# DidItWork/Sigma-Zero

Measured on AMD Instinct MI355X. Metric: MCTS simulations/sec (self-play), higher is better.
Workload: dtype bf16

## Files before the change

### sigma-zero_amd/csrc/sz_nn.hip

```cpp
#include "sz_nn_common.h"

#ifndef NN_EXPLICIT_WAIT
#define NN_EXPLICIT_WAIT 2
#endif
#ifndef NN_TAPGAP
#define NN_TAPGAP 1
#endif


template <int CIN, int NTAPS, int WGB, bool PROBE16 = false>
__device__ __forceinline__ void conv_kloop(const unsigned char* lds, const uint4* __restrict__ w, f32x16 (&acc)[NN_NI][2 * WGB], bool skip) {
    constexpr int PITCH = CIN * 2 + 16;
    constexpr int KSTEPS = CIN / 16;
    constexpr int ZERO_ROW = WGB * 64;
    constexpr int NI = NN_NI, NJ = 2 * WGB;
    constexpr int RING = 4, PF = RING - 1;
    constexpr int TOTAL_KS = NTAPS * KSTEPS;
    constexpr int W_KSTEP_STRIDE = 8 * 64;
    const int lane = threadIdx.x & 63, wave = threadIdx.x >> 6;
    const int p32 = lane & 31, h = lane >> 5;
    const uint4* wbase = w + (size_t)(wave * NI) * 64 + lane;
#pragma unroll
    for (int i = 0; i < NI; i++)
#pragma unroll
        for (int j = 0; j < NJ; j++)
#pragma unroll
            for (int r = 0; r < 16; r++) acc[i][j][r] = 0.f;
    uint4 aring[RING][NI];
#pragma unroll
    for (int s = 0; s < PF; s++)
#pragma unroll
        for (int i = 0; i < NI; i++) aring[s][i] = wbase[(size_t)s * W_KSTEP_STRIDE + i * 64];
    auto tap_addr = [&](int tap, int j) -> int {
        const int dy = (NTAPS == 9) ? tap / 3 - 1 : 0, dx = (NTAPS == 9) ? tap % 3 - 1 : 0;
        int pos = (j & 1) * 32 + p32;
        int y = (pos >> 3) + dy, x = (pos & 7) + dx;
        bool ok = (unsigned)y < 8u && (unsigned)x < 8u;
        int row = ok ? ((j >> 1) * 64 + y * 8 + x) : ZERO_ROW;
        return row * PITCH + h * 16;
    };
    int bcur[NJ], bnxt[NJ];
    bf16x8 bfrag[2][NJ];
#pragma unroll
    for (int j = 0; j < NJ; j++) { bcur[j] = tap_addr(0, j); bnxt[j] = bcur[j]; bfrag[0][j] = *(const bf16x8*)(lds + bcur[j]); }
    for (int tap = 0; tap < (skip ? 0 : NTAPS); tap++) {
        if (tap + 1 < NTAPS) {
#pragma unroll
            for (int j = 0; j < NJ; j++) bnxt[j] = tap_addr(tap + 1, j);
        }
#pragma unroll
        for (int kc = 0; kc < KSTEPS; kc++) {
            const int ks = tap * KSTEPS + kc;
            if (ks + PF < TOTAL_KS) {
#pragma unroll
                for (int i = 0; i < NI; i++) aring[(kc + PF) & (RING - 1)][i] = wbase[(size_t)(ks + PF) * W_KSTEP_STRIDE + i * 64];
            }
            if (kc + 1 < KSTEPS) {
#pragma unroll
                for (int j = 0; j < NJ; j++) bfrag[(kc + 1) & 1][j] = *(const bf16x8*)(lds + bcur[j] + (kc + 1) * 32);
            } else if (tap + 1 < NTAPS) {
#pragma unroll
                for (int j = 0; j < NJ; j++) bfrag[(kc + 1) & 1][j] = *(const bf16x8*)(lds + bnxt[j]);
            }
            asm volatile("" ::: "memory");
            __builtin_amdgcn_sched_barrier(0);
#pragma unroll
            for (int i = 0; i < NI; i++) {
                bf16x8 a = __builtin_bit_cast(bf16x8, aring[kc & (RING - 1)][i]);
#pragma unroll
                for (int j = 0; j < NJ; j++) {
                    if constexpr (PROBE16) {
#pragma unroll
                        for (int q = 0; q < 2; q++) {
                            f32x4 c4 = {acc[i][j][8 * q], acc[i][j][8 * q + 1], acc[i][j][8 * q + 2], acc[i][j][8 * q + 3]};
                            c4 = __builtin_amdgcn_mfma_f32_16x16x32_bf16(a, bfrag[kc & 1][j], c4, 0, 0, 0);
                            acc[i][j][8 * q] = c4[0]; acc[i][j][8 * q + 1] = c4[1]; acc[i][j][8 * q + 2] = c4[2]; acc[i][j][8 * q + 3] = c4[3];
                        }
                    } else {
                        acc[i][j] = __builtin_amdgcn_mfma_f32_32x32x16_bf16(a, bfrag[kc & 1][j], acc[i][j], 0, 0, 0);
                    }
                }
            }
            __builtin_amdgcn_sched_barrier(0);
        }
#pragma unroll
        for (int j = 0; j < NJ; j++) bcur[j] = bnxt[j];
    }
}

template <int WGB>
__device__ __forceinline__ void acc_to_lds(unsigned char* lds, const f32x16 (&acc)[NN_NI][2 * WGB], const float* __restrict__ bias, bool relu) {
    constexpr int OPITCH = NN_COUT * 2 + 16;
    const int lane = threadIdx.x & 63, wave = threadIdx.x >> 6;
    const int p32 = lane & 31, h = lane >> 5;
#pragma unroll
    for (int j = 0; j < 2 * WGB; j++) {
        const int row = (j >> 1) * 64 + (j & 1) * 32 + p32;
#pragma unroll
        for (int i = 0; i < NN_NI; i++) {
#pragma unroll
            for (int g = 0; g < 4; g++) {
                const int co = (wave * NN_NI + i) * 32 + 8 * g + 4 * h;
                f32x4 b4 = *(const f32x4*)(bias + co);
                float v0 = acc[i][j][4 * g + 0] + b4[0], v1 = acc[i][j][4 * g + 1] + b4[1];
                float v2 = acc[i][j][4 * g + 2] + b4[2], v3 = acc[i][j][4 * g + 3] + b4[3];
                if (relu) { v0 = fmaxf(v0, 0.f); v1 = fmaxf(v1, 0.f); v2 = fmaxf(v2, 0.f); v3 = fmaxf(v3, 0.f); }
                uint2 o; o.x = pack_bf16x2(v0, v1); o.y = pack_bf16x2(v2, v3);
                *(uint2*)(lds + row * OPITCH + co * 2) = o;
            }
        }
    }
}

template <int WGB, int PAD = 16, bool NT = false, bool NTS = NT>
__device__ __forceinline__ void lds_to_out(const unsigned char* lds, const uint16_t* __restrict__ res, uint16_t* __restrict__ out, int board0, int n_boards, bool relu) {
    constexpr int OPITCH = NN_COUT * 2 + PAD;
    constexpr int OUT_CHUNKS = WGB * 64 * 32;
    const int tid = threadIdx.x;
    const int valid = min(WGB, n_boards - board0) * 64 * 32;
    const uint4* res4 = res ? (const uint4*)(res + (size_t)board0 * 64 * NN_COUT) : nullptr;
    uint4* out4 = (uint4*)(out + (size_t)board0 * 64 * NN_COUT);
#pragma unroll 4
    for (int c = tid; c < OUT_CHUNKS; c += 256) {
        if (c >= valid) break;
        uint4 v = *(const uint4*)(lds + (c >> 5) * OPITCH + (c & 31) * 16);
        if (!res4 && !relu) {
            if (NTS) st_stream(out4 + c, v); else out4[c] = v;
            continue;
        }
        float f[8] = {bf16_lo(v.x), bf16_hi(v.x), bf16_lo(v.y), bf16_hi(v.y), bf16_lo(v.z), bf16_hi(v.z), bf16_lo(v.w), bf16_hi(v.w)};
        if (res4) {
            uint4 r = NT ? ld_stream(res4 + c) : res4[c];
            f[0] += bf16_lo(r.x); f[1] += bf16_hi(r.x); f[2] += bf16_lo(r.y); f[3] += bf16_hi(r.y);
            f[4] += bf16_lo(r.z); f[5] += bf16_hi(r.z); f[6] += bf16_lo(r.w); f[7] += bf16_hi(r.w);
        }
        if (relu) {
#pragma unroll
            for (int k = 0; k < 8; k++) f[k] = fmaxf(f[k], 0.f);
        }
        uint4 o;
        o.x = pack_bf16x2(f[0], f[1]); o.y = pack_bf16x2(f[2], f[3]); o.z = pack_bf16x2(f[4], f[5]); o.w = pack_bf16x2(f[6], f[7]);
        if (NTS) st_stream(out4 + c, o); else out4[c] = o;
    }
}


template <int RING>
__device__ __forceinline__ void conv_prefetch16(const uint4* __restrict__ w, uint4 (&aring)[RING][4]) {
    const int lane = threadIdx.x & 63, wave = threadIdx.x >> 6;
    const uint32_t wlane = (uint32_t)((wave * 4) * 64 + lane) * 16u;
    const WSrc wr = wfrag_rsrc(w);
#pragma unroll
    for (int s = 0; s < RING - 1; s++)
#pragma unroll
        for (int i = 0; i < 4; i++) aring[s][i] = ld_wfrag(wr, (size_t)s * (16 * 64), wlane + i * 1024);
    asm volatile("" ::: "memory");
    __builtin_amdgcn_sched_barrier(0);
}


template <int CIN, int NTAPS, int WGB, int RING = 2, bool PREFETCHED = false, int ABL = 0 ,
          bool ACCUM = false ,
          class E = ElemBF16 ,
          class EPI = std::nullptr_t >
__device__ __forceinline__ void conv_kloop16(const unsigned char* lds, const uint4* __restrict__ w, f32x4 (&acc)[4][4 * WGB], bool skip, bool wprobe = false,
                                             uint4 (*ring_in)[4] = nullptr, const int img_off = 0 ,
                                             const float* __restrict__ bias = nullptr ,
                                             const int* addr_tab = nullptr ,
                                             EPI epi0 = EPI()) {
    constexpr int PITCH = CIN * 2 + NN_PAD16;
    constexpr int KSTEPS = CIN / 32;
    constexpr int NI = 4, NJ = 4 * WGB, NH = NJ / 2;
    constexpr int TOTAL_KS = NTAPS * KSTEPS;
    const int W_KSTEP_STRIDE = wprobe ? 0 : 16 * 64;
    const int lane = threadIdx.x & 63, wave = threadIdx.x >> 6;
    const int p16 = lane & 15, kg = lane >> 4;
    const uint32_t wlane = (uint32_t)((wave * NI) * 64 + lane) * 16u;
    const WSrc wr = wfrag_rsrc(w);
    f32x4 binit[NI];
#pragma unroll
    for (int i = 0; i < NI; i++) binit[i] = bias ? *(const f32x4*)(bias + (wave * NI + i) * 16 + 4 * kg) : f32x4{0.f, 0.f, 0.f, 0.f};
    constexpr bool PEEL = RING == 4;
    constexpr bool SKIPROWS = PEEL && NTAPS == 9 && WGB == 2 && !(ABL & 4) && NN_ROWSKIP;
    if ((skip || !PEEL) && !ACCUM) {
#pragma unroll
        for (int i = 0; i < NI; i++)
#pragma unroll
            for (int j = 0; j < NJ; j++) acc[i][j] = binit[i];
    } else if (SKIPROWS && !ACCUM) {
#pragma unroll
        for (int i = 0; i < NI; i++) acc[i][0] = binit[i];
    }
    constexpr int PF = RING - 1;
    static_assert(KSTEPS % RING == 0, "ring slots must be compile-time indices");
    uint4 aring[RING][NI];
#pragma unroll
    for (int s = 0; s < PF; s++)
#pragma unroll
        for (int i = 0; i < NI; i++) {
            if constexpr (PREFETCHED) aring[s][i] = ring_in[s][i];
            else aring[s][i] = ld_wfrag(wr, (size_t)s * W_KSTEP_STRIDE, wlane + i * 1024);
        }
    auto tap_addr = [&](int tap, int j) -> int {
        return addr_tab ? addr_tab[(tap * NJ + j) * 64 + lane] : conv_tap_addr16<PITCH, NTAPS, WGB>(tap, j, p16, kg);
    };
    constexpr int TABPITCH = NN_COUT * 2 + NN_PAD16;
    constexpr bool CONVERT = PITCH != TABPITCH;
    auto tab_convert = [&](int rel) -> int {
        if constexpr (!CONVERT) return rel;
        else {
            const int row = (int)__umulhi((unsigned)rel, 7895161u);
            return rel >= WGB * 64 * TABPITCH ? rel - WGB * 64 * (TABPITCH - PITCH) : rel - row * (TABPITCH - PITCH);
        }
    };
    const int lds_base = (int)(uint32_t)(uintptr_t)lds;
    auto abs_addr = [&](int rel) -> int {
        int a = lds_base + img_off + rel;
        asm volatile("" : "+v"(a));
        return a;
    };
    auto LD = [](int addr) -> bf16x8 { return *(const __attribute__((address_space(3))) bf16x8*)(uint32_t)addr; };
    int bcur[NJ], bnxt[NJ];
    bf16x8 bfrag[2][NH];
#pragma unroll
    for (int j = 0; j < NJ; j++) { bnxt[j] = addr_tab ? tab_convert(tap_addr(0, j)) : tap_addr(0, j); bcur[j] = abs_addr(bnxt[j]); }
#pragma unroll
    for (int j = 0; j < NH; j++)
        if (!(SKIPROWS && j == 0)) bfrag[0][j] = LD(bcur[j]);
    auto tap_body = [&](const int tap, auto first_tag, auto skip_tag) {
        constexpr bool FIRST = decltype(first_tag)::value;
        constexpr int SK = decltype(skip_tag)::value;
        constexpr bool TAPGAP = NN_TAPGAP && PEEL && NN_ILV && NH + NJ <= NI * (NH - 1);
        const bool in_gaps = TAPGAP && addr_tab != nullptr;
        if (tap + 1 < NTAPS && !in_gaps) {
#pragma unroll
            for (int j = 0; j < NJ; j++) bnxt[j] = addr_tab ? tab_convert(tap_addr(tap + 1, j)) : tap_addr(tap + 1, j);
        }
#pragma unroll
        for (int kc = 0; kc < KSTEPS; kc++) {
            const int ks = tap * KSTEPS + kc;
#pragma unroll
            for (int hs = 0; hs < 2; hs++) {
                if (!NN_ILV) {
                    if (hs == 0 && ks + PF < TOTAL_KS) {
#pragma unroll
                        for (int i = 0; i < NI; i++) aring[(kc + PF) & (RING - 1)][i] = ld_wfrag(wr, (size_t)(ks + PF) * W_KSTEP_STRIDE, wlane + i * 1024);
                    }
                    if (hs == 0) {
#pragma unroll
                        for (int j = 0; j < NH; j++) if (!(SK == 2 && j == NH - 1)) bfrag[1][j] = LD(bcur[NH + j] + kc * 64);
                    } else if (kc + 1 < KSTEPS) {
#pragma unroll
                        for (int j = 0; j < NH; j++) if (!(SK == 1 && j == 0)) bfrag[0][j] = LD(bcur[j] + (kc + 1) * 64);
                    } else if (tap + 1 < NTAPS) {
#pragma unroll
                        for (int j = 0; j < NH; j++) if (!(SK == 1 && j == 0 && tap + 1 < 3)) bfrag[0][j] = LD(abs_addr(bnxt[j]));
                    }
                    asm volatile("" ::: "memory");
                    __builtin_amdgcn_sched_barrier(0);
                }
#pragma unroll
                for (int i = 0; i < NI; i++) {
                    bf16x8 a = __builtin_bit_cast(bf16x8, aring[kc & (RING - 1)][i]);
#pragma unroll
                    for (int j = 0; j < NH; j++) {
                        const bool idle_hs = (SK == 1 && hs == 0) || (SK == 2 && hs == 1);
                        const bool idle = idle_hs && j == (SK == 1 ? 0 : NH - 1);
                        if (!idle) acc[i][hs * NH + j] = E::mfma(a, bfrag[hs][j], (FIRST && kc == 0) ? binit[i] : acc[i][hs * NH + j]);
                        if (NN_ILV && !idle) {
                            const int NR = idle_hs ? NH - 1 : NH, m = i * NR + (idle_hs && SK == 1 ? j - 1 : j);
                            if (m < NH) {
                                if ((ABL & 2) || (SK == 2 && hs == 0 && m == NH - 1)) {}
                                else if (hs == 0) bfrag[1][m] = LD(bcur[NH + m] + kc * 64);
                                else if (kc + 1 < KSTEPS) { if (!(SK == 1 && m == 0)) bfrag[0][m] = LD(bcur[m] + (kc + 1) * 64); }
                                else if (tap + 1 < NTAPS) { if (!(SK == 1 && m == 0 && tap + 1 < 3)) bfrag[0][m] = LD(abs_addr(bnxt[m])); }
                            } else if (m < NH + NI && hs == 0) {
                                if (ABL & 1) {}
                                else if (ks + PF < TOTAL_KS)
                                    aring[(kc + PF) & (RING - 1)][m - NH] = ld_wfrag(wr, (size_t)(ks + PF) * W_KSTEP_STRIDE, wlane + (m - NH) * 1024);
                            } else if (TAPGAP && hs == 1 && m >= NH && m < NH + NJ) {
                                if (in_gaps) {
                                    if (kc == 0) bnxt[m - NH] = tap_addr(tap + 1 < NTAPS ? tap + 1 : tap, m - NH);
                                    else if (CONVERT && kc == 1) bnxt[m - NH] = tab_convert(bnxt[m - NH]);
                                    else if (kc == KSTEPS - 1) bcur[m - NH] = abs_addr(bnxt[m - NH]);
                                }
                            }
#if NN_EXPLICIT_WAIT
                            if (PEEL && m == NI * NR - 1) {
                                if (NN_EXPLICIT_WAIT >= 2 && hs == 1) __builtin_amdgcn_s_waitcnt(0x0078);
                                else __builtin_amdgcn_s_waitcnt(0xC07F);
                            }
#endif
                            asm volatile("" ::: "memory");
                            __builtin_amdgcn_sched_barrier(0);
                        }
                    }
                }
                __builtin_amdgcn_sched_barrier(0);
            }
        }
        if (!in_gaps) {
#pragma unroll
            for (int j = 0; j < NJ; j++) bcur[j] = abs_addr(bnxt[j]);
        }
    };
    constexpr bool SPLIT = !std::is_same<EPI, std::nullptr_t>::value && NTAPS == 9 && NN_ILV && PEEL && KSTEPS % RING == 0;
    auto last_tap_split = [&]() {
        if constexpr (SPLIT) {
            constexpr int tap = NTAPS - 1;
#pragma unroll
            for (int kc = 0; kc < KSTEPS; kc++) {
                const int ks = tap * KSTEPS + kc;
#pragma unroll
                for (int i = 0; i < NI; i++) {
                    bf16x8 a = __builtin_bit_cast(bf16x8, aring[kc & (RING - 1)][i]);
#pragma unroll
                    for (int j = 0; j < NH; j++) {
                        acc[i][j] = E::mfma(a, bfrag[kc & 1][j], acc[i][j]);
                        const int m = i * NH + j;
                        if (m < NH) {
                            if (ABL & 2) {}
                            else if (kc + 1 < KSTEPS) bfrag[(kc + 1) & 1][m] = LD(bcur[m] + (kc + 1) * 64);
                            else if (!(SKIPROWS && m == NH - 1)) bfrag[(kc + 1) & 1][m] = LD(bcur[NH + m]);
                        } else if (m < NH + NI) {
                            const int vks = ks + PF, wks = vks < TOTAL_KS ? vks : vks - KSTEPS;
                            if (!(ABL & 1)) aring[(kc + PF) & (RING - 1)][m - NH] = ld_wfrag(wr, (size_t)wks * W_KSTEP_STRIDE, wlane + (m - NH) * 1024);
                        } else if (kc == KSTEPS - 1 && (m == 2 * NH || m == 3 * NH)) {
                            epi0(m == 2 * NH ? 0 : 1, -1);
                        }
#if NN_EXPLICIT_WAIT >= 2
                        if (m == NI * NH - 1) __builtin_amdgcn_s_waitcnt(0x0078);
#endif
                        asm volatile("" ::: "memory");
                        __builtin_amdgcn_sched_barrier(0);
                    }
                }
            }
#pragma unroll
            for (int kc = 0; kc < KSTEPS; kc++) {
#pragma unroll
                for (int i = 0; i < NI; i++) {
                    bf16x8 a = __builtin_bit_cast(bf16x8, aring[kc & (RING - 1)][i]);
#pragma unroll
                    for (int j = 0; j < NH; j++) {
                        if (!(SKIPROWS && j == NH - 1))
                            acc[i][NH + j] = E::mfma(a, bfrag[kc & 1][j], acc[i][NH + j]);
                        const int m = i * NH + j;
                        if (m < NH) {
                            if (!(ABL & 2) && kc + 1 < KSTEPS && !(SKIPROWS && m == NH - 1)) bfrag[(kc + 1) & 1][m] = LD(bcur[NH + m] + (kc + 1) * 64);
                        } else if (m < NH + NI) {
                            if (!(ABL & 1) && kc + PF < KSTEPS)
                                aring[(kc + PF) & (RING - 1)][m - NH] = ld_wfrag(wr, (size_t)(tap * KSTEPS + kc + PF) * W_KSTEP_STRIDE, wlane + (m - NH) * 1024);
                        } else {
                            const int p = 2 * kc + (m >= 3 * NH ? 1 : 0);
                            if (p < NI * NH) epi0(p, (m - 2 * NH) & 3);
                        }
                        asm volatile("" ::: "memory");
                        __builtin_amdgcn_sched_barrier(0);
                    }
                }
            }
        }
    };
    if (!skip) {
        using SK0 = std::integral_constant<int, 0>;
        if constexpr (SKIPROWS) {
            using SK1 = std::integral_constant<int, 1>; using SK2 = std::integral_constant<int, 2>;
            tap_body(0, std::integral_constant<bool, !ACCUM>{}, SK1{});
            for (int tap = 1; tap < 3; tap++) tap_body(tap, std::false_type{}, SK1{});
            for (int tap = 3; tap < 6; tap++) tap_body(tap, std::false_type{}, SK0{});
            for (int tap = 6; tap < (SPLIT ? NTAPS - 1 : NTAPS); tap++) tap_body(tap, std::false_type{}, SK2{});
            last_tap_split();
        } else if constexpr (PEEL) {
            tap_body(0, std::integral_constant<bool, !ACCUM>{}, SK0{});
            for (int tap = 1; tap < (SPLIT ? NTAPS - 1 : NTAPS); tap++) tap_body(tap, std::false_type{}, SK0{});
            last_tap_split();
        } else {
            for (int tap = 0; tap < NTAPS; tap++) tap_body(tap, std::false_type{}, SK0{});
        }
    }
}

#ifndef NN_ONE_RING
#define NN_ONE_RING 4
#endif
#ifndef NN_ONE_WHOT
#define NN_ONE_WHOT 0
#endif
template <int ABL = 0, class E = ElemBF16>
__device__ __forceinline__ void conv_kloop16_one(const unsigned char* lds, const uint4* __restrict__ w, f32x4 (&acc)[4][4], uint4 (*ring_in)[4] , const int img_off,
                                                 const float* __restrict__ bias, const int* addr_tab) {
    constexpr int KSTEPS = NN_COUT / 32, NI = 4, NJ = 4, NTAPS = 9, RING = NN_ONE_RING, PF = RING - 1, TOTAL_KS = NTAPS * KSTEPS;
    constexpr int W_KSTEP_STRIDE = NN_ONE_WHOT ? 0 : 16 * 64;
    static_assert(KSTEPS % RING == 0, "ring slots must be compile-time indices");
    const int lane = threadIdx.x & 63, wave = threadIdx.x >> 6, kg = lane >> 4;
    const uint32_t wlane = (uint32_t)((wave * NI) * 64 + lane) * 16u;
    const WSrc wr = wfrag_rsrc(w);
    f32x4 binit[NI];
#pragma unroll
    for (int i = 0; i < NI; i++) binit[i] = *(const f32x4*)(bias + (wave * NI + i) * 16 + 4 * kg);
    uint4 aring[RING][NI];
#pragma unroll
    for (int s_ = 0; s_ < PF; s_++)
#pragma unroll
        for (int i = 0; i < NI; i++) aring[s_][i] = ring_in[s_][i];
    const int lds_base = (int)(uint32_t)(uintptr_t)lds;
    auto abs_addr = [&](int rel) -> int {
        int a = lds_base + img_off + rel;
        asm volatile("" : "+v"(a));
        return a;
    };
    auto LD = [](int addr) -> bf16x8 { return *(const __attribute__((address_space(3))) bf16x8*)(uint32_t)addr; };
    int bcur[NJ], bnxt[NJ];
    bf16x8 bfrag[2][NJ];
#pragma unroll
    for (int j = 0; j < NJ; j++) { bnxt[j] = addr_tab[j * 64 + lane]; bcur[j] = abs_addr(bnxt[j]); }
#pragma unroll
    for (int j = 0; j < NJ; j++) bfrag[0][j] = LD(bcur[j]);
    auto tap_body = [&](const int tap, auto first_tag) {
        constexpr bool FIRST = decltype(first_tag)::value;
#pragma unroll
        for (int kc = 0; kc < KSTEPS; kc++) {
            const int ks = tap * KSTEPS + kc;
#pragma unroll
            for (int i = 0; i < NI; i++) {
                const bf16x8 a = __builtin_bit_cast(bf16x8, aring[kc & (RING - 1)][i]);
#pragma unroll
                for (int j = 0; j < NJ; j++) {
                    acc[i][j] = E::mfma(a, bfrag[kc & 1][j], (FIRST && kc == 0) ? binit[i] : acc[i][j]);
                    const int m = i * NJ + j;
                    if (m < NJ) {
                        if (ABL & 2) {}
                        else if (kc + 1 < KSTEPS) bfrag[(kc + 1) & 1][m] = LD(bcur[m] + (kc + 1) * 64);
                        else if (tap + 1 < NTAPS) bfrag[(kc + 1) & 1][m] = LD(abs_addr(bnxt[m]));
                    } else if (m < NJ + NI) {
                        if (!(ABL & 1) && ks + PF < TOTAL_KS)
                            aring[(kc + PF) & (RING - 1)][m - NJ] = ld_wfrag(wr, (size_t)(ks + PF) * W_KSTEP_STRIDE, wlane + (m - NJ) * 1024);
                    } else if (m < 2 * NJ + NI) {
                        if (kc == 0) bnxt[m - NJ - NI] = addr_tab[((tap + 1 < NTAPS ? tap + 1 : tap) * NJ + (m - NJ - NI)) * 64 + lane];
                        else if (kc == KSTEPS - 1) bcur[m - NJ - NI] = abs_addr(bnxt[m - NJ - NI]);
                    } else if (m == NI * NJ - 1) {
                        if (RING == 4) __builtin_amdgcn_s_waitcnt(0x0078);
                        else __builtin_amdgcn_s_waitcnt(0x4078);
                    }
                    asm volatile("" ::: "memory");
                    __builtin_amdgcn_sched_barrier(0);
                }
            }
        }
    };
    tap_body(0, std::true_type{});
    for (int tap = 1; tap < NTAPS; tap++) tap_body(tap, std::false_type{});
}

#ifndef NN_EPI_NOCONFLICT
#define NN_EPI_NOCONFLICT 0
#endif
__device__ __forceinline__ int epi_slot16(int row, int co) {
#if NN_EPI_NOCONFLICT
    return ((row >> 3) & 7) * 8192 + (co >> 2) * 128 + (((row >> 6) << 3) | (row & 7)) * 8;
#else
    return row * (NN_COUT * 2 + NN_PAD16) + co * 2;
#endif
}

template <int WGB, class E = ElemBF16> struct EpiTile16 {
    unsigned char* img; const f32x4 (&acc)[4][4 * WGB]; f32x4 tv; uint2 o;
    __device__ __forceinline__ EpiTile16(unsigned char* img_, const f32x4 (&acc_)[4][4 * WGB]) : img(img_), acc(acc_) {}
    __device__ __forceinline__ void operator()(int p, int st) {
        const int i = p / (2 * WGB), j = p % (2 * WGB);
        if (st == 0) tv = acc[i][j];
        else if (st == 1) o.x = relu_bf16x2(E::pack2(tv[0], tv[1]));
        else if (st == 2) o.y = relu_bf16x2(E::pack2(tv[2], tv[3]));
        else if (st == 3) {
            const int lane = threadIdx.x & 63, wave = threadIdx.x >> 6;
            const int row = tile_row<WGB>(j, lane & 15), co = (wave * 4 + i) * 16 + 4 * (lane >> 4);
            *(uint2*)(img + epi_slot16(row, co)) = o;
        }
    }
};
template <int WGB, class E = ElemBF16> struct EpiResidual16 {
    unsigned char* img; const f32x4 (&acc)[4][4 * WGB]; f32x4 tv; uint2 o; uint2 rr[3];
    __device__ __forceinline__ EpiResidual16(unsigned char* img_, const f32x4 (&acc_)[4][4 * WGB]) : img(img_), acc(acc_) {}
    __device__ __forceinline__ uint2* slot(int p) const {
        const int i = p / (2 * WGB), j = p % (2 * WGB);
        const int lane = threadIdx.x & 63, wave = threadIdx.x >> 6;
        const int row = tile_row<WGB>(j, lane & 15), co = (wave * 4 + i) * 16 + 4 * (lane >> 4);
        return (uint2*)(img + epi_slot16(row, co));
    }
    __device__ __forceinline__ void operator()(int p, int st) {
        const int i = p / (2 * WGB), j = p % (2 * WGB);
        if (st == -1) rr[p % 3] = *slot(p);
        else if (st == 0) { tv = acc[i][j]; if (p + 2 < 8 * WGB) rr[(p + 2) % 3] = *slot(p + 2); }
        else if (st == 1) o.x = relu_bf16x2(E::pack2(tv[0] + E::lo(rr[p % 3].x), tv[1] + E::hi(rr[p % 3].x)));
        else if (st == 2) o.y = relu_bf16x2(E::pack2(tv[2] + E::lo(rr[p % 3].y), tv[3] + E::hi(rr[p % 3].y)));
        else if (st == 3) *slot(p) = o;
    }
};

template <int WGB, class E = ElemBF16>
__device__ __forceinline__ void acc_tile_to_lds16(unsigned char* lds, const f32x4 (&acc)[4][4 * WGB], int i, int j, bool relu) {
    constexpr int OPITCH = NN_COUT * 2 + NN_PAD16;
    const int lane = threadIdx.x & 63, wave = threadIdx.x >> 6;
    const int row = tile_row<WGB>(j, lane & 15), co = (wave * 4 + i) * 16 + 4 * (lane >> 4);
    const f32x4 v = acc[i][j];
    uint2 o;
    o.x = E::pack2(v[0], v[1]);
    o.y = E::pack2(v[2], v[3]);
    if (relu) { o.x = relu_bf16x2(o.x); o.y = relu_bf16x2(o.y); }
    *(uint2*)(lds + epi_slot16(row, co)) = o;
}
template <int WGB, class E = ElemBF16>
__device__ __forceinline__ void acc_tile_residual16(unsigned char* xlds, const f32x4 (&acc)[4][4 * WGB], int i, int j) {
    constexpr int OPITCH = NN_COUT * 2 + NN_PAD16;
    const int lane = threadIdx.x & 63, wave = threadIdx.x >> 6;
    const int row = tile_row<WGB>(j, lane & 15), co = (wave * 4 + i) * 16 + 4 * (lane >> 4);
    const f32x4 v = acc[i][j];
    uint2* px = (uint2*)(xlds + epi_slot16(row, co));
    const uint2 r = *px;
    uint2 o;
    o.x = relu_bf16x2(E::pack2(v[0] + E::lo(r.x), v[1] + E::hi(r.x)));
    o.y = relu_bf16x2(E::pack2(v[2] + E::lo(r.y), v[3] + E::hi(r.y)));
    *px = o;
}

template <int WGB, class E = ElemBF16>
__device__ __forceinline__ void acc_to_lds16(unsigned char* lds, const f32x4 (&acc)[4][4 * WGB], const float* __restrict__ bias, bool relu) {
    constexpr int OPITCH = NN_COUT * 2 + NN_PAD16;
    const int lane = threadIdx.x & 63, wave = threadIdx.x >> 6;
    const int p16 = lane & 15, kg = lane >> 4;
#pragma unroll
    for (int j = 0; j < 4 * WGB; j++) {
        const int row = tile_row<WGB>(j, p16);
#pragma unroll
        for (int i = 0; i < 4; i++) {
            const int co = (wave * 4 + i) * 16 + 4 * kg;
            f32x4 v = acc[i][j];
            if (bias) v += *(const f32x4*)(bias + co);
            uint2 o;
            o.x = E::pack2(v[0], v[1]);
            o.y = E::pack2(v[2], v[3]);
            if (relu) { o.x = relu_bf16x2(o.x); o.y = relu_bf16x2(o.y); }
            *(uint2*)(lds + row * OPITCH + co * 2) = o;
        }
    }
}

__device__ __forceinline__ void phase_stagger(int flags, int n_cu) {
    const int stagger = (flags >> 8) & 0xFF;
    if (!stagger) return;
    bool second = false;
    if (flags & 32) second = ((int)blockIdx.x >= n_cu && (int)blockIdx.x < 2 * n_cu);
    if (flags & 64) second = ((int)blockIdx.x < 2 * n_cu) && ((__builtin_amdgcn_s_getreg(0x1804) & 1) != 0);
    if (__builtin_amdgcn_readfirstlane((int)second))
        for (int i = 0; i < stagger; i++) __builtin_amdgcn_s_sleep(127);
}

template <int CIN, int NTAPS, int WGB >
__global__ __launch_bounds__(256, (WGB == 2 ? 2 : 1)) void k_conv_bf16(const uint16_t* __restrict__ in, const uint4* __restrict__ w, const float* __restrict__ bias,
                                                      const uint16_t* __restrict__ res, uint16_t* __restrict__ out, int n_boards, int flags, int n_cu) {
    extern __shared__ __attribute__((aligned(16))) unsigned char lds[];
    const int board0 = blockIdx.x * WGB;
    stage_tile<CIN, WGB>(lds, in, board0, n_boards, (flags & 2) != 0);
    __syncthreads();
    if (WGB == 2) phase_stagger(flags, n_cu);
    f32x16 acc[NN_NI][2 * WGB];
    if (CIN == 256 && NTAPS == 9 && WGB == 2 && (flags & 0x20000)) conv_kloop<CIN, NTAPS, WGB, true>(lds, w, acc, (flags & 8) != 0);
    else conv_kloop<CIN, NTAPS, WGB>(lds, w, acc, (flags & 8) != 0);
    __syncthreads();
    if (!((flags & 4) && acc[0][0][0] != 12345.f)) acc_to_lds<WGB>(lds, acc, bias, false);
    __syncthreads();
    if (!(flags & 4)) lds_to_out<WGB>(lds, res, out, board0, n_boards, (flags & 1) != 0);
}

template <int WGB>
__global__ __launch_bounds__(256, (WGB == 2 ? 2 : 1)) void k_block_bf16(const uint16_t* __restrict__ in, const uint4* __restrict__ w1, const float* __restrict__ b1,
                                                       const uint4* __restrict__ w2, const float* __restrict__ b2, uint16_t* __restrict__ out,
                                                       int n_boards, int flags, int n_cu) {
    extern __shared__ __attribute__((aligned(16))) unsigned char lds[];
// ... 277 lines not shown
    float inv = 1.0f;
    if (do_softmax) {
        for (int off = 32; off >= 1; off >>= 1) mx = fmaxf(mx, __shfl_xor(mx, off));
        if (lane == 0) red[wave * 2] = mx;
        __syncthreads();
        mx = fmaxf(red[wave * 2], red[(wave ^ 1) * 2]);
        float sum = 0.f;
#pragma unroll
        for (int i = 0; i < 5; i++)
#pragma unroll
            for (int r = 0; r < 4; r++) {
                const int co = i * 16 + 4 * kg + r;
#pragma unroll
                for (int j = 0; j < 2; j++) {
                    const float e = co < 73 ? __expf(pa[i][j][r] - mx) : 0.f;
                    pa[i][j][r] = e;
                    sum += e;
                }
            }
        for (int off = 32; off >= 1; off >>= 1) sum += __shfl_xor(sum, off);
        if (lane == 0) red[wave * 2 + 1] = sum;
        __syncthreads();
        inv = 1.0f / (red[(wave & 2) * 2 + 1] + red[((wave & 2) + 1) * 2 + 1]);
    }
    if (board0 + pboard < n_boards) {
        float* pb = probs + (size_t)(board0 + pboard) * 4672;
#pragma unroll
        for (int i = 0; i < 5; i++)
#pragma unroll
            for (int r = 0; r < 4; r++) {
                const int co = i * 16 + 4 * kg + r;
                if (co < 73) {
#pragma unroll
                    for (int j = 0; j < 2; j++) pb[co * 64 + (j0 + j) * 16 + p16] = pa[i][j][r] * inv;
                }
            }
    }
}

template <int WGB>
__device__ __forceinline__ void acc_residual_inplace16(unsigned char* xlds, const f32x4 (&acc)[4][4 * WGB], const float* __restrict__ bias) {
    constexpr int OPITCH = NN_COUT * 2 + NN_PAD16;
    const int lane = threadIdx.x & 63, wave = threadIdx.x >> 6;
    const int p16 = lane & 15, kg = lane >> 4;
#pragma unroll
    for (int j = 0; j < 4 * WGB; j++) {
        const int row = tile_row<WGB>(j, p16);
#pragma unroll
        for (int i = 0; i < 4; i++) {
            const int co = (wave * 4 + i) * 16 + 4 * kg;
            f32x4 v = acc[i][j];
            if (bias) v += *(const f32x4*)(bias + co);
            uint2* px = (uint2*)(xlds + row * OPITCH + co * 2);
            const uint2 r = *px;
            uint2 o;
            o.x = relu_bf16x2(pack_bf16x2(v[0] + bf16_lo(r.x), v[1] + bf16_hi(r.x)));
            o.y = relu_bf16x2(pack_bf16x2(v[2] + bf16_lo(r.y), v[3] + bf16_hi(r.y)));
            *px = o;
        }
    }
}

#ifndef NN_STAGGER
#define NN_STAGGER 1
#endif
__device__ __forceinline__ void wave_stagger() {
#if NN_STAGGER
    const int wave = threadIdx.x >> 6;
    if (wave == 1) __builtin_amdgcn_s_sleep(1 * NN_STAGGER);
    else if (wave == 2) __builtin_amdgcn_s_sleep(2 * NN_STAGGER);
    else if (wave == 3) __builtin_amdgcn_s_sleep(3 * NN_STAGGER);
#endif
}

#define NN_MAX_CONVS 40
struct TowerParams {
    const uint4* w[NN_MAX_CONVS];
    const float* b[NN_MAX_CONVS];
    unsigned long long* pace;
    unsigned long long pace_base;
};

#define TILESTAMP(k) do { if (STAMP_ && tile == stamp_tile) { unsigned long long _t = __builtin_amdgcn_s_memtime(); if ((threadIdx.x & 63) == 0) stamps[8192 + (size_t)(blockIdx.x * 4 + (threadIdx.x >> 6)) * 8 + (k)] = _t; } } while (0)
#define TSTAMP(k) do { if (STAMP_ && stamp_now) { unsigned long long _t = __builtin_amdgcn_s_memtime(); if ((threadIdx.x & 63) == 0) stamps[(size_t)(blockIdx.x * 4 + (threadIdx.x >> 6)) * 8 + (k)] = _t; } } while (0)
template <int MODE , class E = ElemBF16 ,
          int WGB = 2 >
__global__ __launch_bounds__(256, 1) void k_tower16_bf16(const uint16_t* __restrict__ planes, TowerParams prm, uint16_t* __restrict__ out, int n_boards, int n_blocks, int flags,
                                                          unsigned long long* __restrict__ stamps) {
    constexpr bool STAMP_ = MODE != 0;
    constexpr int ABL = MODE == 5 ? 4 : (MODE >= 2 ? MODE - 1 : 0);
    constexpr int IMG = WGB * 64 * (NN_COUT * 2 + NN_PAD16) + NN_ZERO16;
    extern __shared__ __attribute__((aligned(16))) unsigned char lds[];
    unsigned char* bufX = lds;
    unsigned char* bufT = lds + IMG;
    const int n_tiles = (n_boards + WGB - 1) / WGB;
    const int stamp_tile = (int)blockIdx.x + (n_tiles > (int)gridDim.x ? (int)gridDim.x : 0);
    for (int c = threadIdx.x; c < NN_ZERO16 / 16; c += 256) {
        *(uint4*)(bufX + WGB * 64 * (NN_COUT * 2 + NN_PAD16) + c * 16) = make_uint4(0, 0, 0, 0);
        *(uint4*)(bufT + WGB * 64 * (NN_COUT * 2 + NN_PAD16) + c * 16) = make_uint4(0, 0, 0, 0);
    }
    int* addr_tab = (int*)(lds + 2 * IMG);
    for (int e = threadIdx.x; e < 9 * 4 * WGB * 64; e += 256)
        addr_tab[e] = conv_tap_addr16<NN_COUT * 2 + NN_PAD16, 9, WGB>(e / (4 * WGB * 64), (e >> 6) % (4 * WGB), e & 15, (e >> 4) & 3);
    f32x4 acc[4][4 * WGB];
    constexpr int TRING = WGB == 1 ? NN_ONE_RING : 4;
    uint4 ring[TRING][4];
    for (int tile = blockIdx.x; tile < n_tiles; tile += gridDim.x) {
        const int board0 = tile * WGB;
        TILESTAMP(0);
        conv_prefetch16<4>(prm.w[0], (uint4 (&)[4][4])ring);
        if (prm.pace && threadIdx.x == 0) {
            const int grp = gridDim.x >> 3, round = (tile - blockIdx.x) / gridDim.x;
            unsigned long long* c = prm.pace + (blockIdx.x & 7);
            const unsigned long long target = prm.pace_base + (unsigned long long)(round + 1) * grp;
            atomicAdd(c, 1ULL);
            for (int spins = 0; spins < 512 && __hip_atomic_load(c, __ATOMIC_RELAXED, __HIP_MEMORY_SCOPE_AGENT) < target; spins++) __builtin_amdgcn_s_sleep(2);
        }
        __syncthreads();
        TILESTAMP(1);
        if (flags & SZ_NN_IN_BITS) stage_tile_bits<WGB, NN_PAD16, E>(bufT, planes, board0, n_boards);
        else stage_tile<128, WGB, NN_PAD16>(bufT, planes, board0, n_boards, false);
        __syncthreads();
        TILESTAMP(2);
        conv_kloop16<128, 9, WGB, 4, true, 0, false, E>(lds, prm.w[0], acc, false, false, ring, IMG, prm.b[0], addr_tab);
        TILESTAMP(3);
        if (n_blocks > 0) conv_prefetch16<TRING>(prm.w[1], ring);
        acc_to_lds16<WGB, E>(bufX, acc, nullptr, true);
        __syncthreads();
        TILESTAMP(4);
        for (int blk = 0; blk < n_blocks; blk++) {
            const bool stamp_now = STAMP_ && blk == 3 && tile == stamp_tile;
            TSTAMP(0);
            wave_stagger();
            auto epi_t = [&](int i, int j) { acc_tile_to_lds16<WGB, E>(bufT, acc, i, j, true); };
            if constexpr (WGB == 2) conv_kloop16<256, 9, WGB, 4, true, ABL, false, E>(bufX, prm.w[1 + 2 * blk], acc, false, false, ring, 0, prm.b[1 + 2 * blk], addr_tab, EpiTile16<WGB, E>(bufT, acc));
            else conv_kloop16_one<ABL, E>(bufX, prm.w[1 + 2 * blk], acc, ring, 0, prm.b[1 + 2 * blk], addr_tab);
            TSTAMP(1);
            conv_prefetch16<TRING>(prm.w[2 + 2 * blk], ring);
#pragma unroll
            for (int j = (WGB == 2 ? 2 * WGB : 0); j < 4 * WGB; j++)
#pragma unroll
                for (int i = 0; i < 4; i++) epi_t(i, j);
            TSTAMP(2);
            __syncthreads();
            TSTAMP(3);
            wave_stagger();
            auto epi_x = [&](int i, int j) { acc_tile_residual16<WGB, E>(bufX, acc, i, j); };
            if constexpr (WGB == 2) conv_kloop16<256, 9, WGB, 4, true, ABL, false, E>(lds, prm.w[2 + 2 * blk], acc, false, false, ring, IMG, prm.b[2 + 2 * blk], addr_tab, EpiResidual16<WGB, E>(bufX, acc));
            else conv_kloop16_one<ABL, E>(lds, prm.w[2 + 2 * blk], acc, ring, IMG, prm.b[2 + 2 * blk], addr_tab);
            TSTAMP(4);
            if (blk + 1 < n_blocks) conv_prefetch16<TRING>(prm.w[3 + 2 * blk], ring);
#pragma unroll
            for (int j = (WGB == 2 ? 2 * WGB : 0); j < 4 * WGB; j++)
#pragma unroll
                for (int i = 0; i < 4; i++) epi_x(i, j);
            TSTAMP(5);
            __syncthreads();
            TSTAMP(6);
            if (STAMP_ && stamp_now && (threadIdx.x & 63) == 0) stamps[(size_t)(blockIdx.x * 4 + (threadIdx.x >> 6)) * 8 + 7] = __builtin_amdgcn_s_memrealtime();
        }
        TILESTAMP(5);
        lds_to_out<WGB, NN_PAD16>(bufX, nullptr, out, board0, n_boards, false);
        TILESTAMP(6);
    }
}


static int default_flags(int flags, int wgb) {
    if (wgb == 2 && !(flags & (32 | 64 | 0xFF00)) && !(flags & 0x10000)) flags |= 32 | (3 << 8);
    return flags;
}

template <int CIN, int NTAPS, int WGB> static int launch_conv(const void* in, const void* w, const float* bias, const void* res, void* out, int n_boards, int flags, hipStream_t s) {
    constexpr int PITCH = CIN * 2 + 16;
    const size_t lds_in = (size_t)(WGB * 64 + 1) * PITCH, lds_out = (size_t)(WGB * 64) * (NN_COUT * 2 + 16);
    const size_t lds = lds_in > lds_out ? lds_in : lds_out;
    static bool attr_flags[NN_MAX_DEVICES] = {};
    bool& attr_set = attr_flags[current_device_slot()];
    if (!attr_set) {
        HIPCHK(hipFuncSetAttribute((const void*)k_conv_bf16<CIN, NTAPS, WGB>, hipFuncAttributeMaxDynamicSharedMemorySize, (int)lds));
        attr_set = true;
    }
    const int grid = (n_boards + WGB - 1) / WGB;
    hipLaunchKernelGGL((k_conv_bf16<CIN, NTAPS, WGB>), dim3(grid), dim3(256), lds, s, (const uint16_t*)in, (const uint4*)w, bias, (const uint16_t*)res,
                       (uint16_t*)out, n_boards, default_flags(flags, WGB), device_cus());
    HIPCHK(hipGetLastError());
    return SZ_OK;
}

template <int WGB> static int launch_block(const void* in, const void* w1, const float* b1, const void* w2, const float* b2, void* out, int n_boards, int flags, hipStream_t s) {
    const size_t lds = (size_t)(WGB * 64 + 1) * (256 * 2 + 16);
    static bool attr_flags[NN_MAX_DEVICES] = {};
    bool& attr_set = attr_flags[current_device_slot()];
    if (!attr_set) {
        HIPCHK(hipFuncSetAttribute((const void*)k_block_bf16<WGB>, hipFuncAttributeMaxDynamicSharedMemorySize, (int)lds));
        attr_set = true;
    }
    const int grid = (n_boards + WGB - 1) / WGB;
    hipLaunchKernelGGL((k_block_bf16<WGB>), dim3(grid), dim3(256), lds, s, (const uint16_t*)in, (const uint4*)w1, b1, (const uint4*)w2, b2, (uint16_t*)out,
                       n_boards, default_flags(flags, WGB), device_cus());
    HIPCHK(hipGetLastError());
    return SZ_OK;
}

template <int CIN, int NTAPS> static int launch_conv16(const void* in, const void* w, const float* bias, const void* res, void* out, int n_boards, int flags, hipStream_t s) {
    constexpr int WGB = 2, PITCH = CIN * 2 + NN_PAD16;
    const size_t lds_in = (size_t)(WGB * 64) * PITCH + NN_ZERO16, lds_out = (size_t)(WGB * 64) * (NN_COUT * 2 + NN_PAD16);
    const size_t lds = lds_in > lds_out ? lds_in : lds_out;
    static bool attr_flags[NN_MAX_DEVICES] = {};
    bool& attr_set = attr_flags[current_device_slot()];
    if (!attr_set) {
        HIPCHK(hipFuncSetAttribute((const void*)k_conv16_bf16<CIN, NTAPS, WGB>, hipFuncAttributeMaxDynamicSharedMemorySize, (int)lds));
        attr_set = true;
    }
    hipLaunchKernelGGL((k_conv16_bf16<CIN, NTAPS, WGB>), dim3((n_boards + WGB - 1) / WGB), dim3(256), lds, s, (const uint16_t*)in, (const uint4*)w, bias,
                       (const uint16_t*)res, (uint16_t*)out, n_boards, default_flags(flags, WGB), device_cus());
    HIPCHK(hipGetLastError());
    return SZ_OK;
}
template <int WGB> static int launch_block16(const void* in, const void* w1, const float* b1, const void* w2, const float* b2, void* out, int n_boards, int flags, hipStream_t s) {
    const size_t lds = (size_t)(WGB * 64) * (256 * 2 + NN_PAD16) + NN_ZERO16;
    static bool attr_flags[NN_MAX_DEVICES] = {};
    bool& attr_set = attr_flags[current_device_slot()];
    if (!attr_set) {
        HIPCHK(hipFuncSetAttribute((const void*)k_block16_bf16<WGB>, hipFuncAttributeMaxDynamicSharedMemorySize, (int)lds));
        attr_set = true;
    }
    hipLaunchKernelGGL((k_block16_bf16<WGB>), dim3((n_boards + WGB - 1) / WGB), dim3(256), lds, s, (const uint16_t*)in, (const uint4*)w1, b1, (const uint4*)w2, b2,
                       (uint16_t*)out, n_boards, default_flags(flags, WGB), device_cus());
    HIPCHK(hipGetLastError());
    return SZ_OK;
}

template <class E> static int pack_weights16_impl(const float* w_in, int32_t cin_real, int32_t cin_padded, int32_t ksize, uint16_t* out) {
    if (!w_in || !out || (ksize != 1 && ksize != 3) || cin_padded % 32 || cin_real > cin_padded) return SZ_ERR_INVALID;
    const int taps = ksize * ksize, ksteps = cin_padded / 32;
    for (int t = 0; t < taps; t++)
        for (int ks = 0; ks < ksteps; ks++)
            for (int tile = 0; tile < 16; tile++)
                for (int l = 0; l < 64; l++)
                    for (int j = 0; j < 8; j++) {
                        int co = tile * 16 + (l & 15), ci = ks * 32 + 8 * (l >> 4) + j;
                        float v = (ci < cin_real) ? w_in[((size_t)co * cin_real + ci) * taps + t] : 0.f;
                        out[((((size_t)t * ksteps + ks) * 16 + tile) * 64 + l) * 8 + j] = E::from_float(v);
                    }
    return SZ_OK;
}
// ... 261 lines not shown
```

Baseline: 603,400.

## Split last-tap MFMA loop to interleave more epilogue tiles and next-weight prefetch

The final tap's K-steps of the fused residual-block conv are split. The last R k-steps run as two half-column MFMA groups, so the epilogue (ReLU, bf16 pack, LDS store, residual add) for already-finished accumulator tiles interleaves densely with the remaining MFMAs. The prefetch of the next conv's weights moves inside the kernel loop so it follows the MFMAs, and the leftover epilogue no longer runs as a separate serial pass. Epilogue functors now take a tile-index mapping, which adds code complexity and register pressure. Edge timestamp probes are also added, but they are gated by STAMP_.

```diff
diff --git a/sigma-zero_amd/csrc/sz_nn.hip b/sigma-zero_amd/csrc/sz_nn.hip
--- a/sigma-zero_amd/csrc/sz_nn.hip
+++ b/sigma-zero_amd/csrc/sz_nn.hip
@@ -5,6 +5,15 @@
 #endif
 #ifndef NN_TAPGAP
 #define NN_TAPGAP 1
+#endif
+#ifndef NN_EPISPLIT
+#define NN_EPISPLIT 3
+#endif
+#ifndef NN_EPIDENSE
+#define NN_EPIDENSE 2
+#endif
+#ifndef NN_EPIDENSE2
+#define NN_EPIDENSE2 NN_EPIDENSE
 #endif
 
 
@@ -162,12 +171,14 @@
 template <int CIN, int NTAPS, int WGB, int RING = 2, bool PREFETCHED = false, int ABL = 0 ,
           bool ACCUM = false ,
           class E = ElemBF16 ,
-          class EPI = std::nullptr_t >
+          class EPI = std::nullptr_t ,
+          class AFTER = std::nullptr_t >
 __device__ __forceinline__ void conv_kloop16(const unsigned char* lds, const uint4* __restrict__ w, f32x4 (&acc)[4][4 * WGB], bool skip, bool wprobe = false,
                                              uint4 (*ring_in)[4] = nullptr, const int img_off = 0 ,
                                              const float* __restrict__ bias = nullptr ,
                                              const int* addr_tab = nullptr ,
-                                             EPI epi0 = EPI()) {
+                                             EPI epi0 = EPI(), const uint4* __restrict__ w_next = nullptr ,
+                                             AFTER after_mma = AFTER()) {
     constexpr int PITCH = CIN * 2 + NN_PAD16;
     constexpr int KSTEPS = CIN / 32;
     constexpr int NI = 4, NJ = 4 * WGB, NH = NJ / 2;
@@ -305,6 +316,30 @@
         }
     };
     constexpr bool SPLIT = !std::is_same<EPI, std::nullptr_t>::value && NTAPS == 9 && NN_ILV && PEEL && KSTEPS % RING == 0;
+    constexpr int R = (SPLIT && NN_EPISPLIT > 0 && NN_EPISPLIT < KSTEPS && NN_EPISPLIT <= RING) ? NN_EPISPLIT : 0;
+    constexpr int KB = KSTEPS - R, NG = NH / 2, NSK = (SKIPROWS && R) ? NI : 0;
+    constexpr int NQ_A = NI * NH + NSK, NQ_B1 = NQ_A + NI * NG, NQ = NI * NJ;
+    constexpr int NB2 = NH - NG - (SKIPROWS ? 1 : 0);
+    struct TileIJ { int i, j; };
+    auto epi_tile = [](int q) -> TileIJ {
+        if (R == 0 || q < NI * NH) return {q / NH, q % NH};
+        if (q < NQ_A) return {q - NI * NH, NJ - 1};
+        if (q < NQ_B1) return {(q - NQ_A) / NG, NH + (q - NQ_A) % NG};
+        return {(q - NQ_B1) / NB2, NH + NG + (q - NQ_B1) % NB2};
+    };
+    constexpr int EPI_NQ = R ? NQ : NI * NH;
+    constexpr int FA = NI * NH - NH - NI, FB2 = NI * NB2 - NB2;
+    auto fb1 = [](int kc) { return NI * NG - NG - (kc + PF < KSTEPS ? NI : 0); };
+    auto b1_before = [&](int kc) { int c = 0; for (int k = KB; k < kc; k++) c += fb1(k); return c; };
+    auto imin = [](int a, int b) { return a < b ? a : b; };
+    const int E1 = imin(KB * FA, 4 * NQ_A);
+    const int E2 = imin(E1 + NN_EPIDENSE * b1_before(KSTEPS), 4 * NQ_A);
+    const int E3 = imin(E2 + NN_EPIDENSE2 * (KSTEPS - KB) * FB2, 4 * NQ_B1);
+    auto epi_op = [&](int c, int ready) {
+        if constexpr (SPLIT) {
+            if (c < 4 * ready) epi0(c >> 2, c & 3, EPI_NQ, epi_tile);
+        }
+    };
     auto last_tap_split = [&]() {
         if constexpr (SPLIT) {
             constexpr int tap = NTAPS - 1;
@@ -326,7 +361,7 @@
                             const int vks = ks + PF, wks = vks < TOTAL_KS ? vks : vks - KSTEPS;
                             if (!(ABL & 1)) aring[(kc + PF) & (RING - 1)][m - NH] = ld_wfrag(wr, (size_t)wks * W_KSTEP_STRIDE, wlane + (m - NH) * 1024);
                         } else if (kc == KSTEPS - 1 && (m == 2 * NH || m == 3 * NH)) {
-                            epi0(m == 2 * NH ? 0 : 1, -1);
+                            epi0(m == 2 * NH ? 0 : 1, -1, EPI_NQ, epi_tile);
                         }
 #if NN_EXPLICIT_WAIT >= 2
                         if (m == NI * NH - 1) __builtin_amdgcn_s_waitcnt(0x0078);
@@ -337,7 +372,7 @@
                 }
             }
 #pragma unroll
-            for (int kc = 0; kc < KSTEPS; kc++) {
+            for (int kc = 0; kc < KB; kc++) {
 #pragma unroll
                 for (int i = 0; i < NI; i++) {
                     bf16x8 a = __builtin_bit_cast(bf16x8, aring[kc & (RING - 1)][i]);
@@ -352,13 +387,62 @@
                             if (!(ABL & 1) && kc + PF < KSTEPS)
                                 aring[(kc + PF) & (RING - 1)][m - NH] = ld_wfrag(wr, (size_t)(tap * KSTEPS + kc + PF) * W_KSTEP_STRIDE, wlane + (m - NH) * 1024);
                         } else {
-                            const int p = 2 * kc + (m >= 3 * NH ? 1 : 0);
-                            if (p < NI * NH) epi0(p, (m - 2 * NH) & 3);
+                            epi_op(kc * FA + m - NH - NI, NQ_A);
                         }
                         asm volatile("" ::: "memory");
                         __builtin_amdgcn_sched_barrier(0);
                     }
                 }
+            }
+            if constexpr (R > 0) {
+#pragma unroll
+                for (int kc = KB; kc < KSTEPS; kc++) {
+#pragma unroll
+                    for (int i = 0; i < NI; i++) {
+                        bf16x8 a = __builtin_bit_cast(bf16x8, aring[kc & (RING - 1)][i]);
+#pragma unroll
+                        for (int j = 0; j < NG; j++) {
+                            acc[i][NH + j] = E::mfma(a, bfrag[kc & 1][j], acc[i][NH + j]);
+                            const int m = i * NG + j;
+                            if (m < NG) {
+                                if (!(ABL & 2) && kc + 1 < KSTEPS) bfrag[(kc + 1) & 1][m] = LD(bcur[NH + m] + (kc + 1) * 64);
+                            } else if (m < NG + NI && kc + PF < KSTEPS) {
+                                if (!(ABL & 1)) aring[(kc + PF) & (RING - 1)][m - NG] = ld_wfrag(wr, (size_t)(tap * KSTEPS + kc + PF) * W_KSTEP_STRIDE, wlane + (m - NG) * 1024);
+                            } else {
+                                const int f = m - NG - (kc + PF < KSTEPS ? NI : 0);
+#pragma unroll
+                                for (int e = 0; e < NN_EPIDENSE; e++) epi_op(E1 + NN_EPIDENSE * (b1_before(kc) + f) + e, NQ_A);
+                            }
+                            asm volatile("" ::: "memory");
+                            __builtin_amdgcn_sched_barrier(0);
+                        }
+                    }
+                }
+#pragma unroll
+                for (int kc = KB; kc < KSTEPS; kc++) {
+#pragma unroll
+                    for (int i = 0; i < NI; i++) {
+                        bf16x8 a = __builtin_bit_cast(bf16x8, aring[kc & (RING - 1)][i]);
+#pragma unroll
+                        for (int jj = 0; jj < NB2; jj++) {
+                            const int j = NG + jj;
+                            acc[i][NH + j] = E::mfma(a, bfrag[kc & 1][j], acc[i][NH + j]);
+                            const int m = i * NB2 + jj;
+                            if (m < NB2) {
+                                if (!(ABL & 2) && kc + 1 < KSTEPS) bfrag[(kc + 1) & 1][j] = LD(bcur[NH + j] + (kc + 1) * 64);
+                            } else {
+#pragma unroll
+                                for (int e = 0; e < NN_EPIDENSE2; e++) epi_op(E2 + NN_EPIDENSE2 * ((kc - KB) * FB2 + m - NB2) + e, NQ_B1);
+                            }
+                            asm volatile("" ::: "memory");
+                            __builtin_amdgcn_sched_barrier(0);
+                        }
+                    }
+                }
+                if constexpr (!std::is_same<AFTER, std::nullptr_t>::value) after_mma();
+                if (w_next) conv_prefetch16<RING>(w_next, *reinterpret_cast<uint4 (*)[RING][4]>(ring_in));
+#pragma unroll
+                for (int c = E3; c < 4 * NQ; c++) epi_op(c, NQ);
             }
         }
     };
@@ -467,14 +551,14 @@
 template <int WGB, class E = ElemBF16> struct EpiTile16 {
     unsigned char* img; const f32x4 (&acc)[4][4 * WGB]; f32x4 tv; uint2 o;
     __device__ __forceinline__ EpiTile16(unsigned char* img_, const f32x4 (&acc_)[4][4 * WGB]) : img(img_), acc(acc_) {}
-    __device__ __forceinline__ void operator()(int p, int st) {
-        const int i = p / (2 * WGB), j = p % (2 * WGB);
-        if (st == 0) tv = acc[i][j];
+    template <class T> __device__ __forceinline__ void operator()(int q, int st, int nq, T tile) {
+        const auto t = tile(q);
+        if (st == 0) tv = acc[t.i][t.j];
         else if (st == 1) o.x = relu_bf16x2(E::pack2(tv[0], tv[1]));
         else if (st == 2) o.y = relu_bf16x2(E::pack2(tv[2], tv[3]));
         else if (st == 3) {
             const int lane = threadIdx.x & 63, wave = threadIdx.x >> 6;
-            const int row = tile_row<WGB>(j, lane & 15), co = (wave * 4 + i) * 16 + 4 * (lane >> 4);
+            const int row = tile_row<WGB>(t.j, lane & 15), co = (wave * 4 + t.i) * 16 + 4 * (lane >> 4);
             *(uint2*)(img + epi_slot16(row, co)) = o;
         }
     }
@@ -482,19 +566,18 @@
 template <int WGB, class E = ElemBF16> struct EpiResidual16 {
     unsigned char* img; const f32x4 (&acc)[4][4 * WGB]; f32x4 tv; uint2 o; uint2 rr[3];
     __device__ __forceinline__ EpiResidual16(unsigned char* img_, const f32x4 (&acc_)[4][4 * WGB]) : img(img_), acc(acc_) {}
-    __device__ __forceinline__ uint2* slot(int p) const {
-        const int i = p / (2 * WGB), j = p % (2 * WGB);
+    __device__ __forceinline__ uint2* slot(int i, int j) const {
         const int lane = threadIdx.x & 63, wave = threadIdx.x >> 6;
         const int row = tile_row<WGB>(j, lane & 15), co = (wave * 4 + i) * 16 + 4 * (lane >> 4);
         return (uint2*)(img + epi_slot16(row, co));
     }
-    __device__ __forceinline__ void operator()(int p, int st) {
-        const int i = p / (2 * WGB), j = p % (2 * WGB);
-        if (st == -1) rr[p % 3] = *slot(p);
-        else if (st == 0) { tv = acc[i][j]; if (p + 2 < 8 * WGB) rr[(p + 2) % 3] = *slot(p + 2); }
-        else if (st == 1) o.x = relu_bf16x2(E::pack2(tv[0] + E::lo(rr[p % 3].x), tv[1] + E::hi(rr[p % 3].x)));
-        else if (st == 2) o.y = relu_bf16x2(E::pack2(tv[2] + E::lo(rr[p % 3].y), tv[3] + E::hi(rr[p % 3].y)));
-        else if (st == 3) *slot(p) = o;
+    template <class T> __device__ __forceinline__ void operator()(int q, int st, int nq, T tile) {
+        const auto t = tile(q);
+        if (st == -1) rr[q % 3] = *slot(t.i, t.j);
+        else if (st == 0) { tv = acc[t.i][t.j]; if (q + 2 < nq) { const auto u = tile(q + 2); rr[(q + 2) % 3] = *slot(u.i, u.j); } }
+        else if (st == 1) o.x = relu_bf16x2(E::pack2(tv[0] + E::lo(rr[q % 3].x), tv[1] + E::hi(rr[q % 3].x)));
+        else if (st == 2) o.y = relu_bf16x2(E::pack2(tv[2] + E::lo(rr[q % 3].y), tv[3] + E::hi(rr[q % 3].y)));
+        else if (st == 3) *slot(t.i, t.j) = o;
     }
 };
 
@@ -938,6 +1021,7 @@
 };
 
 #define TILESTAMP(k) do { if (STAMP_ && tile == stamp_tile) { unsigned long long _t = __builtin_amdgcn_s_memtime(); if ((threadIdx.x & 63) == 0) stamps[8192 + (size_t)(blockIdx.x * 4 + (threadIdx.x >> 6)) * 8 + (k)] = _t; } } while (0)
+#define EDGESTAMP(k, t) do { if (STAMP_ && threadIdx.x == 0 && blockIdx.x < 256 && (k) < 16) stamps[16384 + (size_t)blockIdx.x * 16 + (k)] = (t); } while (0)
 #define TSTAMP(k) do { if (STAMP_ && stamp_now) { unsigned long long _t = __builtin_amdgcn_s_memtime(); if ((threadIdx.x & 63) == 0) stamps[(size_t)(blockIdx.x * 4 + (threadIdx.x >> 6)) * 8 + (k)] = _t; } } while (0)
 template <int MODE , class E = ElemBF16 ,
           int WGB = 2 >
@@ -951,6 +1035,8 @@
     unsigned char* bufT = lds + IMG;
     const int n_tiles = (n_boards + WGB - 1) / WGB;
     const int stamp_tile = (int)blockIdx.x + (n_tiles > (int)gridDim.x ? (int)gridDim.x : 0);
+    EDGESTAMP(14, __builtin_amdgcn_s_memrealtime());
+    EDGESTAMP(0, __builtin_amdgcn_s_memtime());
     for (int c = threadIdx.x; c < NN_ZERO16 / 16; c += 256) {
         *(uint4*)(bufX + WGB * 64 * (NN_COUT * 2 + NN_PAD16) + c * 16) = make_uint4(0, 0, 0, 0);
         *(uint4*)(bufT + WGB * 64 * (NN_COUT * 2 + NN_PAD16) + c * 16) = make_uint4(0, 0, 0, 0);
@@ -960,7 +1046,9 @@
         addr_tab[e] = conv_tap_addr16<NN_COUT * 2 + NN_PAD16, 9, WGB>(e / (4 * WGB * 64), (e >> 6) % (4 * WGB), e & 15, (e >> 4) & 3);
     f32x4 acc[4][4 * WGB];
     constexpr int TRING = WGB == 1 ? NN_ONE_RING : 4;
+    constexpr bool EPISPLIT = WGB == 2 && NN_EPISPLIT > 0;
     uint4 ring[TRING][4];
+    EDGESTAMP(1, __builtin_amdgcn_s_memtime());
     for (int tile = blockIdx.x; tile < n_tiles; tile += gridDim.x) {
         const int board0 = tile * WGB;
         TILESTAMP(0);
@@ -989,27 +1077,37 @@
             TSTAMP(0);
             wave_stagger();
             auto epi_t = [&](int i, int j) { acc_tile_to_lds16<WGB, E>(bufT, acc, i, j, true); };
-            if constexpr (WGB == 2) conv_kloop16<256, 9, WGB, 4, true, ABL, false, E>(bufX, prm.w[1 + 2 * blk], acc, false, false, ring, 0, prm.b[1 + 2 * blk], addr_tab, EpiTile16<WGB, E>(bufT, acc));
-            else conv_kloop16_one<ABL, E>(bufX, prm.w[1 + 2 * blk], acc, ring, 0, prm.b[1 + 2 * blk], addr_tab);
-            TSTAMP(1);
-            conv_prefetch16<TRING>(prm.w[2 + 2 * blk], ring);
-#pragma unroll
-            for (int j = (WGB == 2 ? 2 * WGB : 0); j < 4 * WGB; j++)
-#pragma unroll
-                for (int i = 0; i < 4; i++) epi_t(i, j);
+            if constexpr (EPISPLIT) {
+                conv_kloop16<256, 9, WGB, 4, true, ABL, false, E>(bufX, prm.w[1 + 2 * blk], acc, false, false, ring, 0, prm.b[1 + 2 * blk], addr_tab, EpiTile16<WGB, E>(bufT, acc),
+                                                                  prm.w[2 + 2 * blk], [&] { TSTAMP(1); });
+            } else {
+                if constexpr (WGB == 2) conv_kloop16<256, 9, WGB, 4, true, ABL, false, E>(bufX, prm.w[1 + 2 * blk], acc, false, false, ring, 0, prm.b[1 + 2 * blk], addr_tab, EpiTile16<WGB, E>(bufT, acc));
+                else conv_kloop16_one<ABL, E>(bufX, prm.w[1 + 2 * blk], acc, ring, 0, prm.b[1 + 2 * blk], addr_tab);
+                TSTAMP(1);
+                conv_prefetch16<TRING>(prm.w[2 + 2 * blk], ring);
+#pragma unroll
+                for (int j = (WGB == 2 ? 2 * WGB : 0); j < 4 * WGB; j++)
+#pragma unroll
+                    for (int i = 0; i < 4; i++) epi_t(i, j);
+            }
             TSTAMP(2);
             __syncthreads();
             TSTAMP(3);
             wave_stagger();
             auto epi_x = [&](int i, int j) { acc_tile_residual16<WGB, E>(bufX, acc, i, j); };
-            if constexpr (WGB == 2) conv_kloop16<256, 9, WGB, 4, true, ABL, false, E>(lds, prm.w[2 + 2 * blk], acc, false, false, ring, IMG, prm.b[2 + 2 * blk], addr_tab, EpiResidual16<WGB, E>(bufX, acc));
-            else conv_kloop16_one<ABL, E>(lds, prm.w[2 + 2 * blk], acc, ring, IMG, prm.b[2 + 2 * blk], addr_tab);
-            TSTAMP(4);
-            if (blk + 1 < n_blocks) conv_prefetch16<TRING>(prm.w[3 + 2 * blk], ring);
-#pragma unroll
-            for (int j = (WGB == 2 ? 2 * WGB : 0); j < 4 * WGB; j++)
-#pragma unroll
-                for (int i = 0; i < 4; i++) epi_x(i, j);
+            if constexpr (EPISPLIT) {
+                conv_kloop16<256, 9, WGB, 4, true, ABL, false, E>(lds, prm.w[2 + 2 * blk], acc, false, false, ring, IMG, prm.b[2 + 2 * blk], addr_tab, EpiResidual16<WGB, E>(bufX, acc),
+                                                                  blk + 1 < n_blocks ? prm.w[3 + 2 * blk] : nullptr, [&] { TSTAMP(4); });
+            } else {
+                if constexpr (WGB == 2) conv_kloop16<256, 9, WGB, 4, true, ABL, false, E>(lds, prm.w[2 + 2 * blk], acc, false, false, ring, IMG, prm.b[2 + 2 * blk], addr_tab, EpiResidual16<WGB, E>(bufX, acc));
+                else conv_kloop16_one<ABL, E>(lds, prm.w[2 + 2 * blk], acc, ring, IMG, prm.b[2 + 2 * blk], addr_tab);
+                TSTAMP(4);
+                if (blk + 1 < n_blocks) conv_prefetch16<TRING>(prm.w[3 + 2 * blk], ring);
+#pragma unroll
+                for (int j = (WGB == 2 ? 2 * WGB : 0); j < 4 * WGB; j++)
+#pragma unroll
+                    for (int i = 0; i < 4; i++) epi_x(i, j);
+            }
             TSTAMP(5);
             __syncthreads();
             TSTAMP(6);
@@ -1018,7 +1116,10 @@
         TILESTAMP(5);
         lds_to_out<WGB, NN_PAD16>(bufX, nullptr, out, board0, n_boards, false);
         TILESTAMP(6);
-    }
+        if (STAMP_) { const int round = (tile - (int)blockIdx.x) / (int)gridDim.x; if (round < 11) EDGESTAMP(2 + round, __builtin_amdgcn_s_memtime()); }
+    }
+    EDGESTAMP(13, __builtin_amdgcn_s_memtime());
+    EDGESTAMP(15, __builtin_amdgcn_s_memrealtime());
 }
 
 
```

Result: no change. 608,000 (median of 6 runs) (+0.8%).
